# facebookresearch/SlowFast

Measured on NVIDIA H100. Metric: clips/sec (fwd+bwd) SlowFast-8x8-R50, higher is better.
Workload: dtype bf16x3-split operands, f32 accumulate/storage

## Files before the change

### slowfast_b200/csrc/conv_igemm.cu

```cuda
#include <algorithm>
#include <cstdint>
#include <cstdio>

#include "../../include/slowfast_b200.h"
#include "ptx.cuh"
#include "runtime.h"

namespace sfb {

constexpr int BLOCK_M = 128;
constexpr int MAX_STAGES = 8;
constexpr int EPI_WARPS = 8;
constexpr int EPI_STAGE_FLOATS = 64;
constexpr int MMA_WARPS = 8;
constexpr int PRODUCER_WARP = MMA_WARPS;
constexpr int EPI_WARP0 = MMA_WARPS + 1;
constexpr int CONV_THREADS = 32 * (MMA_WARPS + 1 + EPI_WARPS);
constexpr int BN_MAX = 128;
constexpr int BLOCK_K = 64;
constexpr int KSTEPS = BLOCK_K / 16;

struct ConvParams {
  CUtensorMap tmA[2];
  CUtensorMap tmB[2];
  int M, oq, op, oz, nb;
  int sw, sh, sd;
  int lw, lh, ld;
  int kw, kh, kd;
  int dw, dh, dd;
  int CK, cpt, n_chunks, cps, k_blocks;
  int Ntot, BN, n_tiles, m_tiles;
  int ksplit;
  int stages;
  int a_tiled;
  uint32_t stage_bytes, chunk_bytes, b_bytes, a_total_bytes, a_plane_bytes;
  uint32_t a_layout, a_sbo, a_lbo;
  uint32_t a_kstep[KSTEPS];
  uint32_t acc_pitch;
  uint32_t off_acc, off_staging, off_red, off_bars;
  float* out;
  long long os_n, os_z, os_p, os_q;
  int accumulate;
  int epi_coalesced;
  float* stats;
};

__device__ __forceinline__ int k_block_begin(const ConvParams& p, int kpart) {
  return kpart * p.k_blocks / p.ksplit;
}

int conv_direct_try(const sfb_conv_desc* d, cudaStream_t stream, int* rc_out);

template <int NSPLIT, int BN>
__global__ void __launch_bounds__(CONV_THREADS, 1) conv_igemm_kernel(const __grid_constant__ ConvParams p) {
  static_assert(BN % 16 == 0 && BN <= BN_MAX, "tile width: a multiple of 16 up to BN_MAX");
  extern __shared__ uint8_t smem_raw[];
  uint8_t* smem = reinterpret_cast<uint8_t*>((reinterpret_cast<uintptr_t>(smem_raw) + 1023) & ~uintptr_t(1023));

  const int warp = threadIdx.x >> 5;
  const int lane = threadIdx.x & 31;

  uint64_t* full = reinterpret_cast<uint64_t*>(smem + p.off_bars);
  uint64_t* empty = full + MAX_STAGES;
  uint64_t* tfull = empty + MAX_STAGES;
  uint64_t* tempty = tfull + 1;
  float* acc_tile = reinterpret_cast<float*>(smem + p.off_acc);

  if (threadIdx.x == 0) {
    for (int s = 0; s < p.stages; ++s) {
      mbar_init(&full[s], 1);
      mbar_init(&empty[s], 32 * MMA_WARPS);
    }
    mbar_init(tfull, 32 * MMA_WARPS);
    mbar_init(tempty, EPI_WARPS);
    fence_mbar_init();
    fence_proxy_async_smem();
  }
  __syncthreads();

  const int total_units = p.m_tiles * p.n_tiles * p.ksplit;

  if (warp == PRODUCER_WARP) {
    if (lane == 0) {
      tma_prefetch_desc(&p.tmA[0]);
      tma_prefetch_desc(&p.tmB[0]);
      if (NSPLIT == 3) {
        tma_prefetch_desc(&p.tmA[1]);
        tma_prefetch_desc(&p.tmB[1]);
      }
    }
    int stage = 0;
    uint32_t phase = 0;
    for (int unit = blockIdx.x; unit < total_units; unit += gridDim.x) {
      const int tile = unit / p.ksplit, kpart = unit - tile * p.ksplit;
      const int mt = tile / p.n_tiles, nt = tile - mt * p.n_tiles;
      const int kb0 = k_block_begin(p, kpart), kb1 = k_block_begin(p, kpart + 1);
      int t = mt * BLOCK_M;
      const int q0 = t % p.oq;
      t /= p.oq;
      const int p0 = t % p.op;
      t /= p.op;
      const int z0 = t % p.oz;
      const int n0 = t / p.oz;
      const int cw = p.lw + q0 * p.sw, ch = p.lh + p0 * p.sh, cd = p.ld + z0 * p.sd;
      for (int kb = kb0; kb < kb1; ++kb) {
        mbar_wait(&empty[stage], phase ^ 1);
        if (elect_one()) {
          const int chunk0 = kb * p.cps;
          const uint32_t bytes = (uint32_t(p.cps) * p.chunk_bytes + p.b_bytes) * (NSPLIT == 3 ? 2u : 1u);
          mbar_expect_tx(&full[stage], bytes);
          uint8_t* st = smem + size_t(stage) * p.stage_bytes;
          for (int j = 0; j < p.cps; ++j) {
            const int idx = chunk0 + j;
            int nn = p.nb, c0 = 0;
            uint16_t ow = 0, oh = 0, od = 0;
            if (idx < p.n_chunks) {
              const int tap = idx / p.cpt;
              c0 = (idx - tap * p.cpt) * p.CK;
              const int tw = tap % p.kw;
              const int t2 = tap / p.kw;
              const int th = t2 % p.kh;
              const int td = t2 / p.kh;
              ow = uint16_t(tw * p.dw);
              oh = uint16_t(th * p.dh);
              od = uint16_t(td * p.dd);
              nn = n0;
            }
            if (p.a_tiled) {
              const int row0 = idx < p.n_chunks ? mt * BLOCK_M : p.m_tiles * BLOCK_M;
              tma_load_2d(st + j * p.chunk_bytes, &p.tmA[0], &full[stage], c0, row0);
              if (NSPLIT == 3) tma_load_2d(st + p.a_plane_bytes + j * p.chunk_bytes, &p.tmA[1], &full[stage], c0, row0);
              continue;
            }
            tma_load_im2col_5d(st + j * p.chunk_bytes, &p.tmA[0], &full[stage], c0, cw, ch, cd, nn, ow, oh, od);
            if (NSPLIT == 3)
              tma_load_im2col_5d(st + p.a_plane_bytes + j * p.chunk_bytes, &p.tmA[1], &full[stage], c0, cw, ch, cd,
                                 nn, ow, oh, od);
          }
          tma_load_2d(st + p.a_total_bytes, &p.tmB[0], &full[stage], kb * 64, nt * BN);
          if (NSPLIT == 3)
            tma_load_2d(st + p.a_total_bytes + p.b_bytes, &p.tmB[1], &full[stage], kb * 64, nt * BN);
        }
        __syncwarp();
        if (++stage == p.stages) {
          stage = 0;
          phase ^= 1;
        }
      }
    }
  } else if (warp < MMA_WARPS) {
    const int g = warp >> 2;
    const uint32_t a_row_off = uint32_t(g) * 8u * p.a_sbo;
    float d[BN / 2];
    int stage = 0;
    uint32_t phase = 0;
    int it = 0;
    for (int unit = blockIdx.x; unit < total_units; unit += gridDim.x, ++it) {
      const int kpart = unit % p.ksplit;
      const int kb0 = k_block_begin(p, kpart), kb1 = k_block_begin(p, kpart + 1);
#pragma unroll
      for (int i = 0; i < BN / 2; ++i) d[i] = 0.f;
      int held = -1;
      for (int kb = kb0; kb < kb1; ++kb) {
        mbar_wait(&full[stage], phase);
        wgmma_fence();
        const uint32_t a_base = smem_u32(smem + size_t(stage) * p.stage_bytes) + a_row_off;
        const uint32_t b_base = smem_u32(smem + size_t(stage) * p.stage_bytes) + p.a_total_bytes;
        const uint64_t a_hi0 = make_smem_desc(a_base, p.a_lbo, p.a_sbo, p.a_layout);
        const uint64_t b_hi0 = make_smem_desc(b_base, 16, 1024, 2);
#pragma unroll
        for (int ks = 0; ks < KSTEPS; ++ks) {
          const uint64_t a_hi = a_hi0 + p.a_kstep[ks];
          const uint64_t b_hi = b_hi0 + uint64_t(ks * 2);
          if (NSPLIT == 3) {
            const uint64_t a_lo = a_hi + (p.a_plane_bytes >> 4);
            const uint64_t b_lo = b_hi + (p.b_bytes >> 4);
            wgmma_m64n<BN>(d, a_lo, b_hi);
            wgmma_m64n<BN>(d, a_hi, b_lo);
          }
          wgmma_m64n<BN>(d, a_hi, b_hi);
        }
        wgmma_commit();
        wgmma_wait<1>();
        if (held >= 0) mbar_arrive(&empty[held]);
        held = stage;
        if (++stage == p.stages) {
          stage = 0;
          phase ^= 1;
        }
      }
      wgmma_wait<0>();
      mbar_arrive(&empty[held]);
      mbar_wait(tempty, (it & 1) ^ 1);
      acc_store<BN>(d, BN, acc_tile + size_t(g) * 64 * p.acc_pitch, int(p.acc_pitch));
      mbar_arrive(tfull);
    }
  } else {
    const int ew = warp - EPI_WARP0;
    const int q = ew & 3;
    const int half = ew >> 2;
    long long* roff_s = reinterpret_cast<long long*>(reinterpret_cast<float*>(smem + p.off_staging) + ew * EPI_STAGE_FLOATS);
    float* red = reinterpret_cast<float*>(smem + p.off_red);
    const int sub = lane >> 2, cq = lane & 3;
    constexpr int nchunks = BN >> 4;
    const float* qtile = acc_tile + size_t(q) * 32 * p.acc_pitch;
    int it = 0;
    for (int unit = blockIdx.x; unit < total_units; unit += gridDim.x, ++it) {
      const int tile = unit / p.ksplit;
      const int acc = it & 1;
      const int mt = tile / p.n_tiles, nt = tile - mt * p.n_tiles;
      const int ncol0 = nt * BN;
      const int row = mt * BLOCK_M + q * 32 + lane;
      const bool rvalid = row < p.M;
      long long roff = 0;
      if (rvalid) {
        int t = row;
        const int oq_ = t % p.oq;
        t /= p.oq;
        const int op_ = t % p.op;
        t /= p.op;
        const int oz_ = t % p.oz;
        const int on_ = t / p.oz;
        roff = on_ * p.os_n + oz_ * p.os_z + op_ * p.os_p + oq_ * p.os_q;
      }
      const uint32_t rmask = __ballot_sync(0xffffffffu, rvalid);
      float* red_w = red + ((size_t(acc) * 4 + q) * BN) * 2;
      roff_s[lane] = roff;
      __syncwarp();
      long long ro[4];
#pragma unroll
      for (int k = 0; k < 4; ++k) ro[k] = roff_s[k * 8 + sub];

      mbar_wait(tfull, it & 1);
      for (int ch = half; ch < nchunks; ch += 2) {
        const int c0 = ch * 16;
        const int limit = min(BN, p.Ntot - ncol0) - c0;
        const bool cvalid = cq * 4 < limit;
        float s4[4] = {0.f, 0.f, 0.f, 0.f}, q4[4] = {0.f, 0.f, 0.f, 0.f};
#pragma unroll
        for (int k = 0; k < 4; ++k) {
          const int r = k * 8 + sub;
          const float4 y = *reinterpret_cast<const float4*>(qtile + size_t(r) * p.acc_pitch + c0 + cq * 4);
          s4[0] += y.x; s4[1] += y.y; s4[2] += y.z; s4[3] += y.w;
          q4[0] = fmaf(y.x, y.x, q4[0]); q4[1] = fmaf(y.y, y.y, q4[1]);
          q4[2] = fmaf(y.z, y.z, q4[2]); q4[3] = fmaf(y.w, y.w, q4[3]);
          if (((rmask >> r) & 1u) && cvalid) {
            float4* dst = reinterpret_cast<float4*>(p.out + ro[k] + ncol0 + c0 + cq * 4);
            if (p.accumulate == 2) {
              asm volatile("red.global.add.v4.f32 [%0], {%1, %2, %3, %4};" ::"l"(dst), "f"(y.x), "f"(y.y), "f"(y.z), "f"(y.w)
                           : "memory");
            } else if (p.accumulate) {
              const float4 o = *dst;
              *dst = make_float4(y.x + o.x, y.y + o.y, y.z + o.z, y.w + o.w);
            } else {
              *dst = y;
            }
          }
        }
        if (p.stats != nullptr) {
#pragma unroll
          for (int i = 0; i < 4; ++i) {
#pragma unroll
            for (int o = 4; o <= 16; o <<= 1) {
              s4[i] += __shfl_xor_sync(0xffffffffu, s4[i], o);
              q4[i] += __shfl_xor_sync(0xffffffffu, q4[i], o);
            }
          }
          if (sub == 0) {
#pragma unroll
            for (int i = 0; i < 4; ++i) {
              const int cl = c0 + cq * 4 + i;
              red_w[cl * 2 + 0] = s4[i];
              red_w[cl * 2 + 1] = q4[i];
            }
          }
        }
      }
      __syncwarp();
      if (lane == 0) mbar_arrive(tempty);
      if (p.stats != nullptr) {
        named_bar_sync(1, 32 * EPI_WARPS);
        const float* rb = red + size_t(acc) * 4 * BN * 2;
        for (int cl = ew * 32 + lane; cl < BN; cl += 32 * EPI_WARPS) {
          const int col = ncol0 + cl;
          if (col < p.Ntot) {
            float s = 0.f, s2 = 0.f;
#pragma unroll
            for (int w = 0; w < 4; ++w) {
              s += rb[(size_t(w) * BN + cl) * 2 + 0];
              s2 += rb[(size_t(w) * BN + cl) * 2 + 1];
            }
            p.stats[size_t(col) * p.m_tiles + mt] = s;
            p.stats[(size_t(p.Ntot) + col) * p.m_tiles + mt] = s2;
          }
        }
      }
    }
  }

}

static int pick_ck(int c) {
  if (c % 64 == 0) return 64;
  if (c % 32 == 0) return 32;
  if (c % 16 == 0) return 16;
  return 8;
}

struct ConvGrid {
  int64_t M;
  int CK, cps, n_chunks, k_blocks, BN, m_tiles, n_tiles;
};
static ConvGrid conv_grid(const sfb_conv_desc* d) {
  ConvGrid g;
  g.M = int64_t(d->n) * d->out_t * d->out_h * d->out_w;
  g.CK = pick_ck(d->c);
  g.cps = BLOCK_K / g.CK;
  g.n_chunks = d->kt * d->kh * d->kw * (d->c / g.CK);
  g.k_blocks = (g.n_chunks + g.cps - 1) / g.cps;
  g.BN = std::min((d->cout + 15) / 16 * 16, BN_MAX);
  g.m_tiles = int((g.M + BLOCK_M - 1) / BLOCK_M);
  g.n_tiles = (d->cout + g.BN - 1) / g.BN;
  return g;
}

static bool rows_regular(const sfb_conv_desc* d) {
  return d->os_h == int64_t(d->out_w) * d->os_w && d->os_t == int64_t(d->out_h) * d->os_h &&
         d->os_n == int64_t(d->out_t) * d->os_t;
}

static int conv_ksplit(const sfb_conv_desc* d, const ConvGrid& g, int P, bool with_stats) {
  const int tiles = g.m_tiles * g.n_tiles;
  if (P <= 0 || d->c <= 8 || 2 * tiles < P) return 1;
  if ((d->accumulate == 0 || with_stats) && !rows_regular(d)) return 1;
  if (with_stats && (d->accumulate != 0 || d->cout % 8 != 0 || d->os_w % 4 != 0)) return 1;
  auto cost = [&](int s) { return double((int64_t(tiles) * s + P - 1) / P) / s * (1.0 + 0.02 * (s - 1)); };
  int best = 1;
  for (int s = 2; s <= 8 && 4 * s <= g.k_blocks; ++s)
    if (cost(s) < cost(best)) best = s;
  return cost(best) < 0.9 * cost(1) ? best : 1;
}

}

using namespace sfb;

extern "C" int64_t sfb_conv_m_tiles(const sfb_conv_desc* d) {
  const ConvGrid g = conv_grid(d);
  int sms = 0;
  if (device_limits(&sms, nullptr) == 0 && conv_ksplit(d, g, sms, true) > 1)
    return sfb_bn_split_stats_tiles(g.M, g.M, 1, d->cout);
  return g.m_tiles;
}

extern "C" int32_t sfb_conv_ksplit(const sfb_conv_desc* d) {
  int sms = 0;
  if (device_limits(&sms, nullptr)) return 1;
  return conv_ksplit(d, conv_grid(d), sms, d->stats != nullptr);
}

extern "C" int sfb_conv_igemm(const sfb_conv_desc* d, void* stream_) {
  cudaStream_t stream = reinterpret_cast<cudaStream_t>(stream_);
  int num_sms = 0, smem_optin = 0;
  if (device_limits(&num_sms, &smem_optin)) return -1;
  if (d->nsplit != 1 && d->nsplit != 3) {
    set_error("sfb_conv_igemm: nsplit must be 1 or 3 (got %d)", d->nsplit);
    return -10;
  }
  if (d->c % 8 != 0 || d->c_pitch % 8 != 0 || d->c <= 0) {
    set_error("sfb_conv_igemm: channel count %d / pitch %lld must be positive multiples of 8", d->c,
              (long long)d->c_pitch);
    return -10;
  }
  if (!d->a_hi || !d->b_hi || !d->out || (d->nsplit == 3 && (!d->a_lo || !d->b_lo))) {
    set_error("sfb_conv_igemm: null operand pointer");
    return -10;
  }
  const int64_t M64 = int64_t(d->n) * d->out_t * d->out_h * d->out_w;
  if (M64 <= 0 || M64 > 0x7fffffffLL || d->cout <= 0) {
    set_error("sfb_conv_igemm: bad output extent M=%lld cout=%d", (long long)M64, d->cout);
    return -10;
  }

  {
    int rc_direct = 0;
    if (conv_direct_try(d, stream, &rc_direct)) return rc_direct;
  }
  ConvParams p;
  memset(&p, 0, sizeof(p));
  p.M = int(M64);
  p.oq = d->out_w;
  p.op = d->out_h;
  p.oz = d->out_t;
  p.nb = d->n;
  p.sw = d->str_w;
  p.sh = d->str_h;
  p.sd = d->str_t;
  p.lw = d->low_w;
  p.lh = d->low_h;
  p.ld = d->low_t;
  p.kw = d->kw;
  p.kh = d->kh;
  p.kd = d->kt;
  p.dw = d->dil_w;
  p.dh = d->dil_h;
  p.dd = d->dil_t;
  const ConvGrid g = conv_grid(d);
  const int taps = d->kt * d->kh * d->kw;
  p.CK = g.CK;
  p.cpt = d->c / p.CK;
  p.n_chunks = g.n_chunks;
  p.cps = g.cps;
  p.k_blocks = g.k_blocks;
  p.Ntot = d->cout;
  p.BN = g.BN;
  p.n_tiles = g.n_tiles;
  p.m_tiles = g.m_tiles;
  p.ksplit = conv_ksplit(d, g, num_sms, d->stats != nullptr);
  p.chunk_bytes = BLOCK_M * p.CK * 2;
  p.b_bytes = p.BN * 128;
  p.a_plane_bytes = (uint32_t(p.cps) * p.chunk_bytes + 1023u) / 1024u * 1024u;
  p.a_total_bytes = p.a_plane_bytes * (d->nsplit == 3 ? 2 : 1);
  p.stage_bytes = p.a_total_bytes + p.b_bytes * (d->nsplit == 3 ? 2 : 1);
  p.stage_bytes = (p.stage_bytes + 1023) / 1024 * 1024;
  switch (p.CK) {
    case 64: p.a_layout = 2; p.a_sbo = 1024; p.a_lbo = 16; break;
    case 32: p.a_layout = 4; p.a_sbo = 512; p.a_lbo = 16; break;
    case 16: p.a_layout = 6; p.a_sbo = 256; p.a_lbo = 16; break;
    default: p.a_layout = 0; p.a_sbo = 128; p.a_lbo = p.chunk_bytes; break;
  }
  for (int ks = 0; ks < KSTEPS; ++ks) {
    const int k0 = ks * 16;
    const uint32_t off = p.CK >= 16 ? uint32_t(k0 / p.CK) * p.chunk_bytes + uint32_t(k0 % p.CK) * 2u
                                    : uint32_t(ks * 2) * p.chunk_bytes;
    p.a_kstep[ks] = off >> 4;
  }
  p.acc_pitch = uint32_t(p.BN) + 4;
  const uint32_t acc_bytes = BLOCK_M * p.acc_pitch * 4;
  const uint32_t tail = acc_bytes + EPI_WARPS * EPI_STAGE_FLOATS * 4 + 2 * 4 * p.BN * 2 * 4 + 256;
  const uint32_t budget = uint32_t(smem_optin) - 1024 - tail;
  p.stages = std::min<int>(MAX_STAGES, budget / p.stage_bytes);
  p.stages = std::min(p.stages, std::max(2, p.k_blocks * 4));
  const int ctas_per_sm = 1;
  if (p.stages < 2) {
    set_error("sfb_conv_igemm: not enough shared memory for 2 pipeline stages (stage=%u B)", p.stage_bytes);
    return -11;
  }
  p.off_acc = p.stages * p.stage_bytes;
  p.off_staging = p.off_acc + acc_bytes;
  p.off_red = p.off_staging + EPI_WARPS * EPI_STAGE_FLOATS * 4;
  p.off_bars = p.off_red + 2 * 4 * p.BN * 2 * 4;
  const uint32_t smem_bytes = p.off_bars + 256 + 1024;
  p.out = d->out;
  p.os_n = d->os_n;
  p.os_z = d->os_t;
  p.os_p = d->os_h;
  p.os_q = d->os_w;
  p.accumulate = p.ksplit > 1 ? 2 : d->accumulate;
  p.epi_coalesced = 1;
  p.stats = p.ksplit > 1 ? nullptr : d->stats;

  const int lower[3] = {d->low_w, d->low_h, d->low_t};
  const int strd[3] = {d->str_w, d->str_h, d->str_t};
  const int upper[3] = {d->low_w + (d->out_w - 1) * d->str_w + 1 - d->w, d->low_h + (d->out_h - 1) * d->str_h + 1 - d->h,
                        d->low_t + (d->out_t - 1) * d->str_t + 1 - d->d};
  const SwizzleBytes aswz = p.CK == 64 ? SWZ_128 : p.CK == 32 ? SWZ_64 : p.CK == 16 ? SWZ_32 : SWZ_NONE;
  p.a_tiled = (taps == 1 && d->str_w == 1 && d->str_h == 1 && d->str_t == 1 && d->low_w == 0 && d->low_h == 0 &&
               d->low_t == 0 && d->out_w == d->w && d->out_h == d->h && d->out_t == d->d)
                  ? 1 : 0;
  int rc;
  if (p.a_tiled)
    rc = make_tmap_2d_bf16(&p.tmA[0], d->a_hi, uint64_t(p.M), uint64_t(d->c), uint64_t(d->c_pitch), BLOCK_M, p.CK, aswz);
  else
    rc = make_tmap_im2col_bf16(&p.tmA[0], d->a_hi, d->n, d->d, d->h, d->w, d->c, d->c_pitch, lower, upper, strd, p.CK,
                               BLOCK_M, aswz);
  if (rc) return rc;
  const uint64_t ktot = uint64_t(taps) * d->c;
  rc = make_tmap_2d_bf16(&p.tmB[0], d->b_hi, d->cout, ktot, ktot, p.BN, 64, SWZ_128);
  if (rc) return rc;
  if (d->nsplit == 3) {
    if (p.a_tiled)
      rc = make_tmap_2d_bf16(&p.tmA[1], d->a_lo, uint64_t(p.M), uint64_t(d->c), uint64_t(d->c_pitch), BLOCK_M, p.CK, aswz);
    else
      rc = make_tmap_im2col_bf16(&p.tmA[1], d->a_lo, d->n, d->d, d->h, d->w, d->c, d->c_pitch, lower, upper, strd,
                                 p.CK, BLOCK_M, aswz);
    if (rc) return rc;
    rc = make_tmap_2d_bf16(&p.tmB[1], d->b_lo, d->cout, ktot, ktot, p.BN, 64, SWZ_128);
    if (rc) return rc;
  }

  if (p.ksplit > 1 && d->accumulate == 0) {
    const size_t width = size_t((d->cout + 3) & ~3) * sizeof(float);
    if (cudaMemset2DAsync(d->out, size_t(d->os_w) * sizeof(float), 0, width, size_t(p.M), stream) != cudaSuccess) {
      set_error("sfb_conv_igemm: zero fill of the split-K output failed: %s", cudaGetErrorString(cudaGetLastError()));
      return -20;
    }
  }
  const int units = p.m_tiles * p.n_tiles * p.ksplit;
  const int grid = std::min(units, num_sms * ctas_per_sm);
  {
    typedef void (*KernelFn)(const ConvParams);
#define SFB_CONV_FNS(S) {conv_igemm_kernel<S, 16>, conv_igemm_kernel<S, 32>, conv_igemm_kernel<S, 48>, \
                         conv_igemm_kernel<S, 64>, conv_igemm_kernel<S, 80>, conv_igemm_kernel<S, 96>, \
                         conv_igemm_kernel<S, 112>, conv_igemm_kernel<S, 128>}
    static const KernelFn fns[2][BN_MAX / 16] = {SFB_CONV_FNS(1), SFB_CONV_FNS(3)};
#undef SFB_CONV_FNS
    static bool attr[2][BN_MAX / 16] = {};
    const int a = d->nsplit == 3 ? 1 : 0, b = p.BN / 16 - 1;
    if (!attr[a][b]) {
      cudaFuncSetAttribute(fns[a][b], cudaFuncAttributeMaxDynamicSharedMemorySize, smem_optin);
      attr[a][b] = true;
    }
    fns[a][b]<<<grid, CONV_THREADS, smem_bytes, stream>>>(p);
  }
  if (int rc = launch_status("sfb_conv_igemm", "grid=%d smem=%u stages=%d BN=%d CK=%d ksplit=%d", grid, smem_bytes,
                             p.stages, p.BN, p.CK, p.ksplit))
    return rc;
  if (p.ksplit > 1 && d->stats != nullptr)
    return sfb_bn_split_stats(d->out, d->os_w, p.M, d->cout, 1, p.M, d->stats, stream);
  return 0;
}
```

### slowfast_b200/csrc/ptx.cuh

```cuda
#pragma once
#include <cstdint>
#include <cuda.h>
#include <cuda_runtime.h>

#include "wgmma.cuh"

namespace sfb {

#ifndef SFB_WATCHDOG_SPINS
#define SFB_WATCHDOG_SPINS (1u << 26)
#endif

__device__ __forceinline__ uint32_t smem_u32(const void* p) {
  return static_cast<uint32_t>(__cvta_generic_to_shared(p));
}

__device__ __forceinline__ bool elect_one() {
  uint32_t pred;
  asm volatile(
      "{\n"
      " .reg .pred p;\n"
      " elect.sync _|p, 0xffffffff;\n"
      " selp.u32 %0, 1, 0, p;\n"
      "}\n"
      : "=r"(pred));
  return pred != 0;
}

__device__ __forceinline__ void mbar_init(uint64_t* bar, uint32_t count) {
  asm volatile("mbarrier.init.shared::cta.b64 [%0], %1;" ::"r"(smem_u32(bar)), "r"(count) : "memory");
}
__device__ __forceinline__ void fence_mbar_init() {
  asm volatile("fence.mbarrier_init.release.cluster;" ::: "memory");
}
__device__ __forceinline__ void fence_proxy_async_smem() {
  asm volatile("fence.proxy.async.shared::cta;" ::: "memory");
}
__device__ __forceinline__ void mbar_expect_tx(uint64_t* bar, uint32_t bytes) {
  asm volatile("mbarrier.arrive.expect_tx.shared::cta.b64 _, [%0], %1;" ::"r"(smem_u32(bar)), "r"(bytes)
               : "memory");
}
__device__ __forceinline__ void mbar_arrive(uint64_t* bar) {
  asm volatile("mbarrier.arrive.shared::cta.b64 _, [%0];" ::"r"(smem_u32(bar)) : "memory");
}
__device__ __forceinline__ bool mbar_try_wait(uint64_t* bar, uint32_t parity) {
  uint32_t ok;
  asm volatile(
      "{\n"
      " .reg .pred p;\n"
      " mbarrier.try_wait.parity.shared::cta.b64 p, [%1], %2;\n"
      " selp.u32 %0, 1, 0, p;\n"
      "}\n"
      : "=r"(ok)
      : "r"(smem_u32(bar)), "r"(parity)
      : "memory");
  return ok != 0;
}
__device__ __forceinline__ void mbar_wait(uint64_t* bar, uint32_t parity) {
  uint32_t spins = 0;
  while (!mbar_try_wait(bar, parity)) {
    if (++spins > SFB_WATCHDOG_SPINS) __trap();
  }
}

__device__ __forceinline__ void tma_prefetch_desc(const CUtensorMap* tm) {
  asm volatile("prefetch.tensormap [%0];" ::"l"(tm) : "memory");
}
__device__ __forceinline__ void tma_load_2d(void* smem, const CUtensorMap* tm, uint64_t* bar, int32_t c0,
                                            int32_t c1) {
  asm volatile(
      "cp.async.bulk.tensor.2d.shared::cluster.global.mbarrier::complete_tx::bytes [%0], [%1, {%3, %4}], [%2];"
      ::"r"(smem_u32(smem)), "l"(tm), "r"(smem_u32(bar)), "r"(c0), "r"(c1)
      : "memory");
}
__device__ __forceinline__ void tma_load_im2col_5d(void* smem, const CUtensorMap* tm, uint64_t* bar, int32_t c,
                                                   int32_t w, int32_t h, int32_t d, int32_t n, uint16_t ow,
                                                   uint16_t oh, uint16_t od) {
  asm volatile(
      "cp.async.bulk.tensor.5d.shared::cluster.global.im2col.mbarrier::complete_tx::bytes"
      " [%0], [%1, {%3, %4, %5, %6, %7}], [%2], {%8, %9, %10};"
      ::"r"(smem_u32(smem)), "l"(tm), "r"(smem_u32(bar)), "r"(c), "r"(w), "r"(h), "r"(d), "r"(n), "h"(ow),
        "h"(oh), "h"(od)
      : "memory");
}

__device__ __forceinline__ void wgmma_fence() { asm volatile("wgmma.fence.sync.aligned;" ::: "memory"); }
__device__ __forceinline__ void wgmma_commit() { asm volatile("wgmma.commit_group.sync.aligned;" ::: "memory"); }
template <int N>
__device__ __forceinline__ void wgmma_wait() {
  asm volatile("wgmma.wait_group.sync.aligned %0;" ::"n"(N) : "memory");
}

__device__ __forceinline__ uint64_t make_smem_desc(uint32_t saddr, uint32_t lbo_bytes, uint32_t sbo_bytes,
                                                   uint32_t layout_type) {
  uint64_t d = 0;
  d |= static_cast<uint64_t>((saddr >> 4) & 0x3FFF);
  d |= static_cast<uint64_t>((lbo_bytes >> 4) & 0x3FFF) << 16;
  d |= static_cast<uint64_t>((sbo_bytes >> 4) & 0x3FFF) << 32;
  d |= static_cast<uint64_t>(layout_type & 6) << 61;
  return d;
}

template <int MAXN>
__device__ __forceinline__ void acc_store(const float* d, int n, float* tile, int pitch) {
  const int t = threadIdx.x & 127;
  const int r = (t >> 5) * 16 + ((t & 31) >> 2), c = 2 * (t & 3);
#pragma unroll
  for (int j = 0; j < MAXN / 8; ++j) {
    if (8 * j < n) {
      *reinterpret_cast<float2*>(tile + r * pitch + 8 * j + c) = make_float2(d[4 * j], d[4 * j + 1]);
      *reinterpret_cast<float2*>(tile + (r + 8) * pitch + 8 * j + c) = make_float2(d[4 * j + 2], d[4 * j + 3]);
    }
  }
}
__device__ __forceinline__ void acc_ld_x16(const float* src, uint32_t (&v)[16]) {
#pragma unroll
  for (int j = 0; j < 4; ++j) {
    const float4 x = reinterpret_cast<const float4*>(src)[j];
    v[4 * j] = __float_as_uint(x.x);
    v[4 * j + 1] = __float_as_uint(x.y);
    v[4 * j + 2] = __float_as_uint(x.z);
    v[4 * j + 3] = __float_as_uint(x.w);
  }
}

__device__ __forceinline__ void named_bar_sync(uint32_t id, uint32_t nthreads) {
  asm volatile("bar.sync %0, %1;" ::"r"(id), "r"(nthreads) : "memory");
}

}
```

Baseline: 181.0.

## Switch conv kernel to ping-pong consumer warpgroups with register-direct epilogue

Replaces the 8 MMA warps plus 8 dedicated epilogue warps, which shared an smem accumulator tile, with two consumer warpgroups. Each owns a full 128-row tile (two m64 accumulators) and alternates units in a ping-pong schedule ordered by named barriers, so one group's epilogue overlaps the other's MMAs. setmaxnreg shifts registers from the producer warpgroup to the consumers. The epilogue writes straight from registers through a small swizzled per-warp staging buffer, and BatchNorm stats come from shuffles. The freed shared memory can go to more pipeline stages, at the cost of higher register pressure and more complex barrier ordering.

```diff
diff --git a/slowfast_b200/csrc/conv_igemm.cu b/slowfast_b200/csrc/conv_igemm.cu
--- a/slowfast_b200/csrc/conv_igemm.cu
+++ b/slowfast_b200/csrc/conv_igemm.cu
@@ -10,15 +10,17 @@
 
 constexpr int BLOCK_M = 128;
 constexpr int MAX_STAGES = 8;
-constexpr int EPI_WARPS = 8;
-constexpr int EPI_STAGE_FLOATS = 64;
-constexpr int MMA_WARPS = 8;
-constexpr int PRODUCER_WARP = MMA_WARPS;
-constexpr int EPI_WARP0 = MMA_WARPS + 1;
-constexpr int CONV_THREADS = 32 * (MMA_WARPS + 1 + EPI_WARPS);
+constexpr int CONV_THREADS = 384;
+constexpr int PRODUCER_REGS = 40;
+constexpr int CONSUMER_REGS = 232;
+constexpr int BAR_ORDER = 1;
+constexpr int BAR_EPI = 3;
 constexpr int BN_MAX = 128;
 constexpr int BLOCK_K = 64;
 constexpr int KSTEPS = BLOCK_K / 16;
+constexpr long long kNoRow = INT64_MIN;
+constexpr uint32_t EPI_SCRATCH = BLOCK_M * 8 + 4 * 8 * 32 * 4;
+static_assert(4 * BN_MAX * 2 * 4 <= 4 * 8 * 32 * 4, "BatchNorm partials fit the staging blocks");
 
 struct ConvParams {
   CUtensorMap tmA[2];
@@ -36,12 +38,10 @@
   uint32_t stage_bytes, chunk_bytes, b_bytes, a_total_bytes, a_plane_bytes;
   uint32_t a_layout, a_sbo, a_lbo;
   uint32_t a_kstep[KSTEPS];
-  uint32_t acc_pitch;
-  uint32_t off_acc, off_staging, off_red, off_bars;
+  uint32_t off_epi, off_bars;
   float* out;
   long long os_n, os_z, os_p, os_q;
   int accumulate;
-  int epi_coalesced;
   float* stats;
 };
 
@@ -50,6 +50,64 @@
 }
 
 int conv_direct_try(const sfb_conv_desc* d, cudaStream_t stream, int* rc_out);
+
+template <int BN, int MODE>
+__device__ __forceinline__ void store_fragment(const float (&d)[2][BN / 2], float* stage, const long long* roff,
+                                               float* out, int ncols) {
+  const int warp = (threadIdx.x >> 5) & 3, lane = threadIdx.x & 31;
+  const int g = lane >> 2, cq = 2 * (lane & 3);
+  const int rr = lane >> 3, c4 = 4 * (lane & 7);
+#pragma unroll
+  for (int rb = 0; rb < 2; ++rb) {
+#pragma unroll
+    for (int h = 0; h < 2; ++h) {
+#pragma unroll
+      for (int cg = 0; cg < (BN + 31) / 32; ++cg) {
+#pragma unroll
+        for (int jj = 0; jj < 4; ++jj) {
+          const int jn = 4 * cg + jj;
+          if (jn < BN / 8)
+            *reinterpret_cast<float2*>(stage + g * 32 + ((8 * jj + cq) ^ (8 * (g & 3)))) =
+                make_float2(d[rb][4 * jn + 2 * h], d[rb][4 * jn + 2 * h + 1]);
+        }
+        __syncwarp();
+        float4 v[2];
+#pragma unroll
+        for (int k = 0; k < 2; ++k) v[k] = *reinterpret_cast<const float4*>(stage + (rr + 4 * k) * 32 + (c4 ^ (8 * rr)));
+        __syncwarp();
+        const int col = 32 * cg + c4;
+        if (col >= ncols) continue;
+        float4* dst[2];
+        bool ok[2];
+#pragma unroll
+        for (int k = 0; k < 2; ++k) {
+          const long long o = roff[64 * rb + 16 * warp + 8 * h + rr + 4 * k];
+          ok[k] = o != kNoRow;
+          dst[k] = reinterpret_cast<float4*>(out + (ok[k] ? o + col : 0));
+        }
+        if (MODE == 1) {
+          float4 o[2];
+#pragma unroll
+          for (int k = 0; k < 2; ++k)
+            if (ok[k]) o[k] = *dst[k];
+#pragma unroll
+          for (int k = 0; k < 2; ++k)
+            if (ok[k]) *dst[k] = make_float4(v[k].x + o[k].x, v[k].y + o[k].y, v[k].z + o[k].z, v[k].w + o[k].w);
+        } else {
+#pragma unroll
+          for (int k = 0; k < 2; ++k) {
+            if (!ok[k]) continue;
+            if (MODE == 2)
+              asm volatile("red.global.add.v4.f32 [%0], {%1, %2, %3, %4};" ::"l"(dst[k]), "f"(v[k].x), "f"(v[k].y),
+                           "f"(v[k].z), "f"(v[k].w) : "memory");
+            else
+              *dst[k] = v[k];
+          }
+        }
+      }
+    }
+  }
+}
 
 template <int NSPLIT, int BN>
 __global__ void __launch_bounds__(CONV_THREADS, 1) conv_igemm_kernel(const __grid_constant__ ConvParams p) {
@@ -57,22 +115,14 @@
   extern __shared__ uint8_t smem_raw[];
   uint8_t* smem = reinterpret_cast<uint8_t*>((reinterpret_cast<uintptr_t>(smem_raw) + 1023) & ~uintptr_t(1023));
 
-  const int warp = threadIdx.x >> 5;
-  const int lane = threadIdx.x & 31;
-
   uint64_t* full = reinterpret_cast<uint64_t*>(smem + p.off_bars);
   uint64_t* empty = full + MAX_STAGES;
-  uint64_t* tfull = empty + MAX_STAGES;
-  uint64_t* tempty = tfull + 1;
-  float* acc_tile = reinterpret_cast<float*>(smem + p.off_acc);
 
   if (threadIdx.x == 0) {
     for (int s = 0; s < p.stages; ++s) {
       mbar_init(&full[s], 1);
-      mbar_init(&empty[s], 32 * MMA_WARPS);
-    }
-    mbar_init(tfull, 32 * MMA_WARPS);
-    mbar_init(tempty, EPI_WARPS);
+      mbar_init(&empty[s], 128);
+    }
     fence_mbar_init();
     fence_proxy_async_smem();
   }
@@ -80,8 +130,10 @@
 
   const int total_units = p.m_tiles * p.n_tiles * p.ksplit;
 
-  if (warp == PRODUCER_WARP) {
-    if (lane == 0) {
+  if (threadIdx.x < 128) {
+    setmaxnreg_dec<PRODUCER_REGS>();
+    if (threadIdx.x >= 32) return;
+    if (threadIdx.x == 0) {
       tma_prefetch_desc(&p.tmA[0]);
       tma_prefetch_desc(&p.tmB[0]);
       if (NSPLIT == 3) {
@@ -148,156 +200,127 @@
         }
       }
     }
-  } else if (warp < MMA_WARPS) {
-    const int g = warp >> 2;
-    const uint32_t a_row_off = uint32_t(g) * 8u * p.a_sbo;
-    float d[BN / 2];
-    int stage = 0;
-    uint32_t phase = 0;
-    int it = 0;
-    for (int unit = blockIdx.x; unit < total_units; unit += gridDim.x, ++it) {
-      const int kpart = unit % p.ksplit;
-      const int kb0 = k_block_begin(p, kpart), kb1 = k_block_begin(p, kpart + 1);
-#pragma unroll
-      for (int i = 0; i < BN / 2; ++i) d[i] = 0.f;
-      int held = -1;
+    return;
+  }
+
+  setmaxnreg_inc<CONSUMER_REGS>();
+  const int c = (threadIdx.x >> 7) - 1;
+  const int t = threadIdx.x & 127, warp = t >> 5, lane = t & 31;
+  const uint32_t a_rb = (8u * p.a_sbo) >> 4;
+  float d[2][BN / 2];
+  int stage = 0;
+  uint32_t phase = 0;
+  for (int j = 0, unit = blockIdx.x; unit < total_units; ++j, unit += gridDim.x) {
+    const int tile = unit / p.ksplit, kpart = unit - tile * p.ksplit;
+    const int kb0 = k_block_begin(p, kpart), kb1 = k_block_begin(p, kpart + 1);
+    if ((j & 1) != c) {
       for (int kb = kb0; kb < kb1; ++kb) {
-        mbar_wait(&full[stage], phase);
-        wgmma_fence();
-        const uint32_t a_base = smem_u32(smem + size_t(stage) * p.stage_bytes) + a_row_off;
-        const uint32_t b_base = smem_u32(smem + size_t(stage) * p.stage_bytes) + p.a_total_bytes;
-        const uint64_t a_hi0 = make_smem_desc(a_base, p.a_lbo, p.a_sbo, p.a_layout);
-        const uint64_t b_hi0 = make_smem_desc(b_base, 16, 1024, 2);
-#pragma unroll
-        for (int ks = 0; ks < KSTEPS; ++ks) {
-          const uint64_t a_hi = a_hi0 + p.a_kstep[ks];
-          const uint64_t b_hi = b_hi0 + uint64_t(ks * 2);
-          if (NSPLIT == 3) {
-            const uint64_t a_lo = a_hi + (p.a_plane_bytes >> 4);
-            const uint64_t b_lo = b_hi + (p.b_bytes >> 4);
-            wgmma_m64n<BN>(d, a_lo, b_hi);
-            wgmma_m64n<BN>(d, a_hi, b_lo);
-          }
-          wgmma_m64n<BN>(d, a_hi, b_hi);
-        }
-        wgmma_commit();
-        wgmma_wait<1>();
-        if (held >= 0) mbar_arrive(&empty[held]);
-        held = stage;
         if (++stage == p.stages) {
           stage = 0;
           phase ^= 1;
         }
       }
-      wgmma_wait<0>();
-      mbar_arrive(&empty[held]);
-      mbar_wait(tempty, (it & 1) ^ 1);
-      acc_store<BN>(d, BN, acc_tile + size_t(g) * 64 * p.acc_pitch, int(p.acc_pitch));
-      mbar_arrive(tfull);
-    }
-  } else {
-    const int ew = warp - EPI_WARP0;
-    const int q = ew & 3;
-    const int half = ew >> 2;
-    long long* roff_s = reinterpret_cast<long long*>(reinterpret_cast<float*>(smem + p.off_staging) + ew * EPI_STAGE_FLOATS);
-    float* red = reinterpret_cast<float*>(smem + p.off_red);
-    const int sub = lane >> 2, cq = lane & 3;
-    constexpr int nchunks = BN >> 4;
-    const float* qtile = acc_tile + size_t(q) * 32 * p.acc_pitch;
-    int it = 0;
-    for (int unit = blockIdx.x; unit < total_units; unit += gridDim.x, ++it) {
-      const int tile = unit / p.ksplit;
-      const int acc = it & 1;
-      const int mt = tile / p.n_tiles, nt = tile - mt * p.n_tiles;
-      const int ncol0 = nt * BN;
-      const int row = mt * BLOCK_M + q * 32 + lane;
-      const bool rvalid = row < p.M;
-      long long roff = 0;
-      if (rvalid) {
-        int t = row;
-        const int oq_ = t % p.oq;
-        t /= p.oq;
-        const int op_ = t % p.op;
-        t /= p.op;
-        const int oz_ = t % p.oz;
-        const int on_ = t / p.oz;
-        roff = on_ * p.os_n + oz_ * p.os_z + op_ * p.os_p + oq_ * p.os_q;
-      }
-      const uint32_t rmask = __ballot_sync(0xffffffffu, rvalid);
-      float* red_w = red + ((size_t(acc) * 4 + q) * BN) * 2;
-      roff_s[lane] = roff;
-      __syncwarp();
-      long long ro[4];
-#pragma unroll
-      for (int k = 0; k < 4; ++k) ro[k] = roff_s[k * 8 + sub];
-
-      mbar_wait(tfull, it & 1);
-      for (int ch = half; ch < nchunks; ch += 2) {
-        const int c0 = ch * 16;
-        const int limit = min(BN, p.Ntot - ncol0) - c0;
-        const bool cvalid = cq * 4 < limit;
-        float s4[4] = {0.f, 0.f, 0.f, 0.f}, q4[4] = {0.f, 0.f, 0.f, 0.f};
-#pragma unroll
-        for (int k = 0; k < 4; ++k) {
-          const int r = k * 8 + sub;
-          const float4 y = *reinterpret_cast<const float4*>(qtile + size_t(r) * p.acc_pitch + c0 + cq * 4);
-          s4[0] += y.x; s4[1] += y.y; s4[2] += y.z; s4[3] += y.w;
-          q4[0] = fmaf(y.x, y.x, q4[0]); q4[1] = fmaf(y.y, y.y, q4[1]);
-          q4[2] = fmaf(y.z, y.z, q4[2]); q4[3] = fmaf(y.w, y.w, q4[3]);
-          if (((rmask >> r) & 1u) && cvalid) {
-            float4* dst = reinterpret_cast<float4*>(p.out + ro[k] + ncol0 + c0 + cq * 4);
-            if (p.accumulate == 2) {
-              asm volatile("red.global.add.v4.f32 [%0], {%1, %2, %3, %4};" ::"l"(dst), "f"(y.x), "f"(y.y), "f"(y.z), "f"(y.w)
-                           : "memory");
-            } else if (p.accumulate) {
-              const float4 o = *dst;
-              *dst = make_float4(y.x + o.x, y.y + o.y, y.z + o.z, y.w + o.w);
-            } else {
-              *dst = y;
-            }
+      continue;
+    }
+    if (j > 0) named_bar_sync(BAR_ORDER + c, 256);
+#pragma unroll
+    for (int i = 0; i < BN / 2; ++i) d[0][i] = d[1][i] = 0.f;
+    int held = -1;
+    for (int kb = kb0; kb < kb1; ++kb) {
+      mbar_wait(&full[stage], phase);
+      wgmma_fence();
+      const uint32_t a_base = smem_u32(smem + size_t(stage) * p.stage_bytes);
+      const uint32_t b_base = a_base + p.a_total_bytes;
+      const uint64_t a_hi0 = make_smem_desc(a_base, p.a_lbo, p.a_sbo, p.a_layout);
+      const uint64_t b_hi0 = make_smem_desc(b_base, 16, 1024, 2);
+#pragma unroll
+      for (int ks = 0; ks < KSTEPS; ++ks) {
+        const uint64_t a_hi = a_hi0 + p.a_kstep[ks];
+        const uint64_t b_hi = b_hi0 + uint64_t(ks * 2);
+        if (NSPLIT == 3) {
+          const uint64_t a_lo = a_hi + (p.a_plane_bytes >> 4);
+          const uint64_t b_lo = b_hi + (p.b_bytes >> 4);
+          wgmma_m64n<BN>(d[0], a_lo, b_hi);
+          wgmma_m64n<BN>(d[1], a_lo + a_rb, b_hi);
+          wgmma_m64n<BN>(d[0], a_hi, b_lo);
+          wgmma_m64n<BN>(d[1], a_hi + a_rb, b_lo);
+        }
+        wgmma_m64n<BN>(d[0], a_hi, b_hi);
+        wgmma_m64n<BN>(d[1], a_hi + a_rb, b_hi);
+      }
+      wgmma_commit();
+      wgmma_wait<1>();
+      if (held >= 0) mbar_arrive(&empty[held]);
+      held = stage;
+      if (++stage == p.stages) {
+        stage = 0;
+        phase ^= 1;
+      }
+    }
+    if (unit + int(gridDim.x) < total_units) named_bar_arrive(BAR_ORDER + (c ^ 1), 256);
+
+    const int mt = tile / p.n_tiles, nt = tile - mt * p.n_tiles;
+    const int ncol0 = nt * BN;
+    uint8_t* epi = smem + p.off_epi + size_t(c) * EPI_SCRATCH;
+    long long* roff_s = reinterpret_cast<long long*>(epi);
+    {
+      int r = mt * BLOCK_M + t;
+      long long off = kNoRow;
+      if (r < p.M) {
+        const int oq_ = r % p.oq;
+        r /= p.oq;
+        const int op_ = r % p.op;
+        r /= p.op;
+        const int oz_ = r % p.oz;
+        const int on_ = r / p.oz;
+        off = on_ * p.os_n + oz_ * p.os_z + op_ * p.os_p + oq_ * p.os_q;
+      }
+      roff_s[t] = off;
+    }
+    named_bar_sync(BAR_EPI + c, 128);
+    const int cq = 2 * (lane & 3);
+    const int ncols = min(BN, ((p.Ntot + 3) & ~3) - ncol0);
+    float* stage_w = reinterpret_cast<float*>(epi + BLOCK_M * 8) + warp * 256;
+    wgmma_wait<0>();
+    mbar_arrive(&empty[held]);
+    if (p.accumulate == 2) store_fragment<BN, 2>(d, stage_w, roff_s, p.out + ncol0, ncols);
+    else if (p.accumulate == 1) store_fragment<BN, 1>(d, stage_w, roff_s, p.out + ncol0, ncols);
+    else store_fragment<BN, 0>(d, stage_w, roff_s, p.out + ncol0, ncols);
+    if (p.stats != nullptr) {
+      float* red = reinterpret_cast<float*>(epi + BLOCK_M * 8);
+      named_bar_sync(BAR_EPI + c, 128);
+#pragma unroll
+      for (int jn = 0; jn < BN / 8; ++jn) {
+        float s[2], q[2];
+#pragma unroll
+        for (int e = 0; e < 2; ++e) {
+          const float a0 = d[0][4 * jn + e], a1 = d[0][4 * jn + 2 + e], a2 = d[1][4 * jn + e], a3 = d[1][4 * jn + 2 + e];
+          s[e] = (a0 + a1) + (a2 + a3);
+          q[e] = fmaf(a0, a0, fmaf(a1, a1, fmaf(a2, a2, a3 * a3)));
+#pragma unroll
+          for (int o = 4; o <= 16; o <<= 1) {
+            s[e] += __shfl_xor_sync(0xffffffffu, s[e], o);
+            q[e] += __shfl_xor_sync(0xffffffffu, q[e], o);
           }
         }
-        if (p.stats != nullptr) {
-#pragma unroll
-          for (int i = 0; i < 4; ++i) {
-#pragma unroll
-            for (int o = 4; o <= 16; o <<= 1) {
-              s4[i] += __shfl_xor_sync(0xffffffffu, s4[i], o);
-              q4[i] += __shfl_xor_sync(0xffffffffu, q4[i], o);
-            }
-          }
-          if (sub == 0) {
-#pragma unroll
-            for (int i = 0; i < 4; ++i) {
-              const int cl = c0 + cq * 4 + i;
-              red_w[cl * 2 + 0] = s4[i];
-              red_w[cl * 2 + 1] = q4[i];
-            }
-          }
-        }
-      }
-      __syncwarp();
-      if (lane == 0) mbar_arrive(tempty);
-      if (p.stats != nullptr) {
-        named_bar_sync(1, 32 * EPI_WARPS);
-        const float* rb = red + size_t(acc) * 4 * BN * 2;
-        for (int cl = ew * 32 + lane; cl < BN; cl += 32 * EPI_WARPS) {
-          const int col = ncol0 + cl;
-          if (col < p.Ntot) {
-            float s = 0.f, s2 = 0.f;
-#pragma unroll
-            for (int w = 0; w < 4; ++w) {
-              s += rb[(size_t(w) * BN + cl) * 2 + 0];
-              s2 += rb[(size_t(w) * BN + cl) * 2 + 1];
-            }
-            p.stats[size_t(col) * p.m_tiles + mt] = s;
-            p.stats[(size_t(p.Ntot) + col) * p.m_tiles + mt] = s2;
-          }
-        }
-      }
-    }
-  }
-
+        if (lane < 4)
+          *reinterpret_cast<float4*>(red + (size_t(warp) * BN + 8 * jn + cq) * 2) = make_float4(s[0], q[0], s[1], q[1]);
+      }
+      named_bar_sync(BAR_EPI + c, 128);
+      const int col = ncol0 + t;
+      if (t < BN && col < p.Ntot) {
+        float s = 0.f, s2 = 0.f;
+#pragma unroll
+        for (int w = 0; w < 4; ++w) {
+          s += red[(size_t(w) * BN + t) * 2 + 0];
+          s2 += red[(size_t(w) * BN + t) * 2 + 1];
+        }
+        p.stats[size_t(col) * p.m_tiles + mt] = s;
+        p.stats[(size_t(p.Ntot) + col) * p.m_tiles + mt] = s2;
+      }
+      named_bar_sync(BAR_EPI + c, 128);
+    }
+  }
 }
 
 static int pick_ck(int c) {
@@ -435,10 +458,8 @@
                                     : uint32_t(ks * 2) * p.chunk_bytes;
     p.a_kstep[ks] = off >> 4;
   }
-  p.acc_pitch = uint32_t(p.BN) + 4;
-  const uint32_t acc_bytes = BLOCK_M * p.acc_pitch * 4;
-  const uint32_t tail = acc_bytes + EPI_WARPS * EPI_STAGE_FLOATS * 4 + 2 * 4 * p.BN * 2 * 4 + 256;
-  const uint32_t budget = uint32_t(smem_optin) - 1024 - tail;
+  const uint32_t epi_bytes = 2u * EPI_SCRATCH;
+  const uint32_t budget = uint32_t(smem_optin) - 1024 - epi_bytes - 256;
   p.stages = std::min<int>(MAX_STAGES, budget / p.stage_bytes);
   p.stages = std::min(p.stages, std::max(2, p.k_blocks * 4));
   const int ctas_per_sm = 1;
@@ -446,10 +467,8 @@
     set_error("sfb_conv_igemm: not enough shared memory for 2 pipeline stages (stage=%u B)", p.stage_bytes);
     return -11;
   }
-  p.off_acc = p.stages * p.stage_bytes;
-  p.off_staging = p.off_acc + acc_bytes;
-  p.off_red = p.off_staging + EPI_WARPS * EPI_STAGE_FLOATS * 4;
-  p.off_bars = p.off_red + 2 * 4 * p.BN * 2 * 4;
+  p.off_epi = p.stages * p.stage_bytes;
+  p.off_bars = p.off_epi + epi_bytes;
   const uint32_t smem_bytes = p.off_bars + 256 + 1024;
   p.out = d->out;
   p.os_n = d->os_n;
@@ -457,7 +476,6 @@
   p.os_p = d->os_h;
   p.os_q = d->os_w;
   p.accumulate = p.ksplit > 1 ? 2 : d->accumulate;
-  p.epi_coalesced = 1;
   p.stats = p.ksplit > 1 ? nullptr : d->stats;
 
   const int lower[3] = {d->low_w, d->low_h, d->low_t};
diff --git a/slowfast_b200/csrc/ptx.cuh b/slowfast_b200/csrc/ptx.cuh
--- a/slowfast_b200/csrc/ptx.cuh
+++ b/slowfast_b200/csrc/ptx.cuh
@@ -127,5 +127,17 @@
 __device__ __forceinline__ void named_bar_sync(uint32_t id, uint32_t nthreads) {
   asm volatile("bar.sync %0, %1;" ::"r"(id), "r"(nthreads) : "memory");
 }
+__device__ __forceinline__ void named_bar_arrive(uint32_t id, uint32_t nthreads) {
+  asm volatile("bar.arrive %0, %1;" ::"r"(id), "r"(nthreads) : "memory");
+}
+
+template <int N>
+__device__ __forceinline__ void setmaxnreg_dec() {
+  asm volatile("setmaxnreg.dec.sync.aligned.u32 %0;" ::"n"(N));
+}
+template <int N>
+__device__ __forceinline__ void setmaxnreg_inc() {
+  asm volatile("setmaxnreg.inc.sync.aligned.u32 %0;" ::"n"(N));
+}
 
 }
```

After: 195.3 (median of 6 runs). +7.8%, better.
